# fircarpediem/LSS2_Multimodal_nu

Measured on AMD Instinct MI355X. Metric: BEV frames/sec (6-cam 352x128 -> 200x200x64), full hot path: CamEncode lift + splat + BevEncode, higher is better.
Workload: dtype bf16; 1 GPU; BASELINE configs[1]: model_BEV_TXT LSS hot path, batch=4/GPU, 6 cams 352x128, D=41, 200x200x64 BEV -> BevEncode -> 200x200x4, trunk (EfficientNet) not included: features are the input; batch_per_gpu=4, global_batch=4, parallelism=dp1 (sample-sharded, no collective), precision=bf16

## Files before the change

lss2_multimodal_nu_amd/csrc/conv_ring.hip:

```cpp
#include <type_traits>

#include "conv_launch.h"
#include "lss_device.h"

namespace {

constexpr int RK_SW = 20, RK_SH = 4;
constexpr int RK_PW = 24, RK_PH = 6;
constexpr int RK_KC = 32;
constexpr int RK_POSB = RK_KC * 2;
constexpr int RK_STRIP_PATCH = RK_PH * RK_PW * RK_POSB;
constexpr int RK_SLAB = 128 * RK_KC * 2;
constexpr int RK_SRC_H = 5, RK_SRC_W = 14;
constexpr int RK_SRC_STRIP = RK_SRC_H * RK_SRC_W * RK_POSB;
constexpr int RK_TH = 2 * RK_SH, RK_TW = 2 * RK_SW;
constexpr int RK_TPW = RK_TW + 2, RK_TPH = RK_TH + 2;
constexpr int RK_TPIECE = (RK_TPH * RK_TPW * 4 + 63) / 64;
constexpr int RK_TSRC_H = 7, RK_TSRC_W = 23;
constexpr int RK_TSRC = RK_TSRC_H * RK_TSRC_W * RK_POSB;
constexpr int RK_TSRC_PIECE = (RK_TSRC_H * RK_TSRC_W * 4 + 63) / 64;

struct RingArgs {
  const unsigned short* x;
  const unsigned short* x2;
  const unsigned char* w;
  const float* scale;
  const float* shift;
  unsigned short* y;
  const float* head_w;
  const float* head_b;
  float* head_out;
  int head_n;
  int B, H, W, Cx, C2, up, Hin, Win, Cin, Cout, relu, wt;
  float ry, rx;
  int SX, SY, nstrips, nblk, nch;
  unsigned long long* stats;
};

__device__ __attribute__((aligned(128))) unsigned char lss_ring_zero_page[128];
__device__ int lss_ring_timeouts;

template <int MODE, bool HEAD, int NSL, bool T22>
struct RingLds {
  static constexpr int RING = 0;
  static constexpr int PATCH = NSL * RK_SLAB;
  static constexpr int PBUF = T22 ? RK_TPIECE * 1024 : 4 * RK_STRIP_PATCH;
  static constexpr int SRC = PATCH + 2 * PBUF;
  static constexpr int HEADX = SRC + (MODE == 1 ? (T22 ? RK_TSRC : 4 * RK_SRC_STRIP) : 0);
  static constexpr int FLAGS = HEADX + (HEAD ? 4 * 80 * 4 * 4 : 0);
  static constexpr int TOTAL = FLAGS + 256;
};
constexpr int F_FULL_W = 0, F_FREE_W = 8, F_FULL_P = 16, F_FREE_P = 18, F_HEAD = 20, F_FULL_S = 24, F_FREE_S = 25;

#define RK_TIMEOUT_COUNTER lss_ring_timeouts
#include "ring_prims.h"

typedef __attribute__((ext_vector_type(2))) __bf16 rk_bf16x2;
__device__ __forceinline__ unsigned int rk_pack_bf2(float lo, float hi) {
  const f32x2 v = {lo, hi};
  return __builtin_bit_cast(unsigned int, __builtin_convertvector(v, rk_bf16x2));
}
__device__ __forceinline__ uint4 rk_blend(const uint4& q00, const uint4& q01, const uint4& q10, const uint4& q11,
                                          float lx, float ly) {
  const float w11 = lx * ly, w10 = ly - w11, w01 = lx - w11, w00 = 1.f - lx - ly + w11;
  const unsigned int* u00 = reinterpret_cast<const unsigned int*>(&q00);
  const unsigned int* u01 = reinterpret_cast<const unsigned int*>(&q01);
  const unsigned int* u10 = reinterpret_cast<const unsigned int*>(&q10);
  const unsigned int* u11 = reinterpret_cast<const unsigned int*>(&q11);
  uint4 out;
  unsigned int* o = reinterpret_cast<unsigned int*>(&out);
#pragma unroll
  for (int i = 0; i < 4; ++i) {
    float lo = __builtin_bit_cast(float, u00[i] << 16) * w00;
    float hi = __builtin_bit_cast(float, u00[i] & 0xffff0000u) * w00;
    lo = __builtin_fmaf(__builtin_bit_cast(float, u01[i] << 16), w01, lo);
    hi = __builtin_fmaf(__builtin_bit_cast(float, u01[i] & 0xffff0000u), w01, hi);
    lo = __builtin_fmaf(__builtin_bit_cast(float, u10[i] << 16), w10, lo);
    hi = __builtin_fmaf(__builtin_bit_cast(float, u10[i] & 0xffff0000u), w10, hi);
    lo = __builtin_fmaf(__builtin_bit_cast(float, u11[i] << 16), w11, lo);
    hi = __builtin_fmaf(__builtin_bit_cast(float, u11[i] & 0xffff0000u), w11, hi);
    o[i] = rk_pack_bf2(lo, hi);
  }
  return out;
}

#ifndef RK_PSLEEP
#define RK_PSLEEP 8
#endif
#ifndef RK_PRIO_C
#define RK_PRIO_C 0
#endif
#ifndef RK_PRIO_P
#define RK_PRIO_P 3
#endif
#ifndef RK_PRIO_W
#define RK_PRIO_W 2
#endif
constexpr int RK_NS = 4;
constexpr int RK_NCONS = 2 * RK_NS;
constexpr int RK_NPATCH = 3;
constexpr int RK_NWAVES = RK_NCONS + 1 + RK_NPATCH;

struct RingTile {
  int nb;
  int b[RK_NS], oy0[RK_NS], ox0[RK_NS];
  bool ok[RK_NS];
};

template <int MODE, bool HEAD, int NSL, bool T22>
__global__ __launch_bounds__(RK_NWAVES * 64, 3) void conv_ring_kernel(RingArgs a) {
  static_assert(!T22 || MODE == 1, "shared tile: fused upsample only");
  using L = RingLds<MODE, HEAD, NSL, T22>;
  constexpr int PW = T22 ? RK_TPW : RK_PW;
  constexpr int LA = NSL - 2;
  static_assert(NSL >= 3 && NSL <= 8, "ring depth");
  static_assert(L::TOTAL <= 160 * 1024, "LDS of one CU");
  __shared__ __attribute__((aligned(1024))) unsigned char smem[L::TOTAL];
  const int tid = threadIdx.x, lane = tid & 63;
  const int wave = __builtin_amdgcn_readfirstlane(tid >> 6);
  const rk_flag_t flags = (rk_flag_t)((__attribute__((address_space(3))) unsigned char*)smem + L::FLAGS);
  if (tid < 64) flags[tid] = 0;
  __syncthreads();
  int st0 = 0, st1 = 0;
#ifdef RK_STATS
#define RK_ST(x) x
  const unsigned long long t_entry = a.stats ? __builtin_amdgcn_s_memrealtime() : 0ull;
  auto write_stats = [&]() {
    if (a.stats != nullptr && lane == 0) {
      unsigned long long* o = a.stats + ((size_t)blockIdx.x * RK_NWAVES + wave) * 6;
      o[0] = (unsigned long long)st0; o[1] = (unsigned long long)st1;
      o[2] = __builtin_amdgcn_s_memrealtime() - t_entry; o[3] = t_entry;
    }
  };
#else
#define RK_ST(x)
  auto write_stats = [&]() {};
#endif

  RingTile T;
  {
    const int t = lss_xcd_order(blockIdx.x, gridDim.x);
    T.nb = t % a.nblk;
    const int quad = t / a.nblk;
    if (T22) {
      const int tx = a.SX >> 1, per = tx * (a.SY >> 1);
      const int b = quad / per, rem = quad - b * per, ty = rem / tx;
#pragma unroll
      for (int s = 0; s < RK_NS; ++s) {
        T.ok[s] = true;
        T.b[s] = b;
        T.oy0[s] = ty * RK_TH + (s >> 1) * RK_SH;
        T.ox0[s] = (rem - ty * tx) * RK_TW + (s & 1) * RK_SW;
      }
    } else {
#pragma unroll
      for (int s = 0; s < RK_NS; ++s) {
        int sid = RK_NS * quad + s;
        T.ok[s] = sid < a.nstrips;
        sid = min(sid, a.nstrips - 1);
        const int per = a.SX * a.SY;
        T.b[s] = sid / per;
        const int rem = sid - T.b[s] * per;
        const int sy = rem / a.SX;
        T.oy0[s] = sy * RK_SH;
        T.ox0[s] = (rem - sy * a.SX) * RK_SW;
      }
    }
  }
  const int nsteps = a.nch * 9;

  if (wave == RK_NCONS) {
    __builtin_amdgcn_s_setprio(RK_PRIO_W);
    const unsigned char* wsrc = a.w + (size_t)T.nb * a.nch * 9 * RK_SLAB + lane * 16;
    int slot = 0, gen = 1, pslot = 0, pgen = 1, inflight = 0;
    auto publish_oldest = [&]() {
      switch (inflight) {
        case 1: lss_wait_vmcnt<0>(); break;
        case 2: lss_wait_vmcnt<8>(); break;
        case 3: lss_wait_vmcnt<16>(); break;
        case 4: lss_wait_vmcnt<24>(); break;
        case 5: lss_wait_vmcnt<32>(); break;
        case 6: lss_wait_vmcnt<40>(); break;
        default: lss_wait_vmcnt<48>(); break;
      }
      rk_set(flags + F_FULL_W + pslot, pgen, lane);
      if (++pslot == NSL) { pslot = 0; ++pgen; }
      --inflight;
    };
    for (int i = 0; i < nsteps; ++i) {
      if (gen > 1) {
        int spins = 0;
        while (rk_peek(flags + F_FREE_W + slot) < RK_NCONS * (gen - 1)) {
          if (inflight > 0) {
            publish_oldest();
          } else {
            __builtin_amdgcn_s_sleep(1);
            ++st0;
            if (++spins > RK_SPIN_LIMIT) {
              if (lane == 0) atomicAdd(&lss_ring_timeouts, 1);
              break;
            }
          }
        }
        asm volatile("" ::: "memory");
      }
      unsigned char* dst = smem + L::RING + slot * RK_SLAB;
#ifndef RK_DIAG_NOWDMA
#pragma unroll
      for (int k = 0; k < 8; ++k) lss_glds16(wsrc + (size_t)i * RK_SLAB + k * 1024, dst + k * 1024);
#endif
      ++inflight;
      if (inflight > LA) publish_oldest();
      if (++slot == NSL) { slot = 0; ++gen; }
    }
    while (inflight > 0) publish_oldest();
    lss_wait_vmcnt<0>();
    write_stats();
    return;
  }

  if (wave > RK_NCONS) {
    __builtin_amdgcn_s_setprio(RK_PRIO_P);
    const int pw = wave - RK_NCONS - 1;
    constexpr int NIT = (T22 ? RK_TPIECE : RK_NS * 9) / RK_NPATCH;
    static_assert(NIT * RK_NPATCH == (T22 ? RK_TPIECE : RK_NS * 9), "pieces split evenly over the patch loaders");
    const int nskip = MODE == 1 ? a.C2 / RK_KC : a.nch;
    const unsigned short* xfull = MODE == 1 ? a.x2 : a.x;
    const int cfull = MODE == 1 ? a.C2 : a.Cx;
    int poff[NIT];
    int g_off[MODE == 1 ? NIT : 1];
    constexpr int NWD = MODE == 1 && T22 ? NIT : 1, NWP = MODE == 1 && !T22 ? NIT : 1;
    float g_lx[NWD], g_ly[NWD];
    unsigned int g_wp[NWP];
    constexpr int SRCW = T22 ? RK_TSRC_W : RK_SRC_W;
    constexpr int NSRCP = T22 ? RK_TSRC_PIECE : RK_NS * 5;
    constexpr int NSRC = MODE == 1 ? (NSRCP + RK_NPATCH - 1) / RK_NPATCH : 1;
    int src_o[NSRC];
#pragma unroll
    for (int k = 0; k < NIT; ++k) {
      const int it = pw + k * RK_NPATCH;
      const int s = T22 ? 0 : it / 9, pos = T22 ? it * 16 + (lane >> 2) : (it % 9) * 16 + (lane >> 2);
      const int prow = pos / PW, pcol = pos - prow * PW;
      const int piece = (lane & 3) ^ ((prow & 1) << 1);
      const int sb = s == 0 ? T.b[0] : s == 1 ? T.b[1] : s == 2 ? T.b[2] : T.b[3];
      const int soy = s == 0 ? T.oy0[0] : s == 1 ? T.oy0[1] : s == 2 ? T.oy0[2] : T.oy0[3];
      const int sox = s == 0 ? T.ox0[0] : s == 1 ? T.ox0[1] : s == 2 ? T.ox0[2] : T.ox0[3];
      const bool sok = s == 0 ? T.ok[0] : s == 1 ? T.ok[1] : s == 2 ? T.ok[2] : T.ok[3];
      const int iy = soy - 1 + prow, ix = sox - 1 + pcol;
      const bool used = T22 ? pos < RK_TPH * RK_TPW : pcol < RK_SW + 2;
      const bool in = sok && used && iy >= 0 && iy < a.Hin && ix >= 0 && ix < a.Win;
      poff[k] = (in && cfull > 0) ? ((sb * a.Hin + iy) * a.Win + ix) * cfull + piece * 8 : -1;
      if (MODE == 1) {
        g_off[k] = 0;
        unsigned int g_w = 0;
        if (in) {
          const int wy0 = (int)(a.ry * (float)max(soy - 1, 0)), wx0 = (int)(a.rx * (float)max(sox - 1, 0));
          const float sy = a.ry * (float)iy, sx = a.rx * (float)ix;
          const int y0 = (int)sy, x0 = (int)sx;
          const unsigned int wy = (unsigned int)((sy - (float)y0) * 65536.f + 0.5f);
          const unsigned int wx = (unsigned int)((sx - (float)x0) * 65536.f + 0.5f);
          g_w = min(wx, 65535u) | (min(wy, 65535u) << 16);
          const int fl = (x0 < a.W - 1 ? 1 : 0) | (y0 < a.H - 1 ? 2 : 0) | 4;
          g_off[k] = ((((y0 - wy0) * SRCW + (x0 - wx0)) * 4 + piece) * 16) | fl;
        }
        if constexpr (T22) {
          g_lx[k] = (float)(g_w & 0xffff) * (1.f / 65536.f);
          g_ly[k] = (float)(g_w >> 16) * (1.f / 65536.f);
        } else {
          g_wp[k] = g_w;
        }
      }
    }
    if (MODE == 1) {
#pragma unroll
      for (int k = 0; k < NSRC; ++k) {
        const int it = pw + k * RK_NPATCH;
        const int s = T22 ? 0 : min(it / 5, RK_NS - 1), q = (T22 ? it : it % 5) * 64 + lane;
        const int pos = min(q >> 2, (T22 ? RK_TSRC_H : RK_SRC_H) * SRCW - 1), part = q & 3;
        const int sr = pos / SRCW, sc = pos - sr * SRCW;
        const int sb = s == 0 ? T.b[0] : s == 1 ? T.b[1] : s == 2 ? T.b[2] : T.b[3];
        const int soy = s == 0 ? T.oy0[0] : s == 1 ? T.oy0[1] : s == 2 ? T.oy0[2] : T.oy0[3];
        const int sox = s == 0 ? T.ox0[0] : s == 1 ? T.ox0[1] : s == 2 ? T.ox0[2] : T.ox0[3];
        const int wy0 = (int)(a.ry * (float)max(soy - 1, 0)), wx0 = (int)(a.rx * (float)max(sox - 1, 0));
        src_o[k] = ((sb * a.H + min(wy0 + sr, a.H - 1)) * a.W + min(wx0 + sc, a.W - 1)) * a.Cx + part * 8;
      }
    }
    auto issue_full = [&](int c, int buf) {
      unsigned char* dst = smem + L::PATCH + buf * L::PBUF;
#pragma unroll
      for (int k = 0; k < NIT; ++k) {
        const void* src = poff[k] >= 0 ? (const void*)(xfull + poff[k] + c * RK_KC) : (const void*)lss_ring_zero_page;
        lss_glds16(src, dst + (pw + k * RK_NPATCH) * 1024);
      }
    };
    if (MODE == 0) {
      issue_full(0, 0);
      if (a.nch > 1) {
        issue_full(1, 1);
        lss_wait_vmcnt<NIT>();
      } else {
        lss_wait_vmcnt<0>();
      }
      rk_add1(flags + F_FULL_P + 0, lane);
      for (int c = 0; c < a.nch; ++c) {
        if (c + 1 < a.nch) {
          lss_wait_vmcnt<0>();
          rk_add1(flags + F_FULL_P + ((c + 1) & 1), lane);
        }
        if (c + 2 < a.nch) {
          st0 += rk_wait_ge<RK_PSLEEP>(flags + F_FREE_P + (c & 1), RK_NCONS * ((c >> 1) + 1));
          issue_full(c + 2, c & 1);
        }
      }
    } else {
      auto issue_src = [&](int c) {
        const int cx = c * RK_KC - a.C2;
#pragma unroll
        for (int k = 0; k < NSRC; ++k) {
          const int it = pw + k * RK_NPATCH;
          if (T22) {
            if (it < RK_TSRC_PIECE && it * 64 + lane < RK_TSRC_H * RK_TSRC_W * 4)
              lss_glds16(a.x + src_o[k] + cx, smem + L::SRC + it * 1024);
          } else if (it < RK_NS * 5 && (it % 5) * 64 + lane < RK_SRC_H * RK_SRC_W * 4) {
            lss_glds16(a.x + src_o[k] + cx, smem + L::SRC + (it / 5) * RK_SRC_STRIP + (it % 5) * 1024);
          }
        }
      };
      auto prepare = [&](int c) {
        if (c < nskip) {
          st0 += rk_wait_ge<RK_PSLEEP>(flags + F_FREE_P + (c & 1), RK_NCONS * (c >> 1));
          issue_full(c, c & 1);
        } else {
          st1 += rk_wait_ge(flags + F_FREE_S, RK_NPATCH * (c - nskip));
          issue_src(c);
        }
      };
      prepare(0);
      for (int c = 0; c < a.nch; ++c) {
        lss_wait_vmcnt<0>();
        if (c >= nskip) {
          rk_add1(flags + F_FULL_S, lane);
          st1 += rk_wait_ge(flags + F_FULL_S, RK_NPATCH * (c - nskip + 1));
          st0 += rk_wait_ge<RK_PSLEEP>(flags + F_FREE_P + (c & 1), RK_NCONS * (c >> 1));
          unsigned char* dst = smem + L::PATCH + (c & 1) * L::PBUF;
          uint4 qa[4], qb[4];
          auto corners = [&](int k, uint4* q) {
            const int it = pw + k * RK_NPATCH;
            const unsigned char* p00 = smem + L::SRC + (T22 ? 0 : (it / 9) * RK_SRC_STRIP) + (g_off[k] & 0xfff0);
            const int dx = (g_off[k] & 1) ? 4 * 16 : 0, dy = (g_off[k] & 2) ? SRCW * 4 * 16 : 0;
            q[0] = *reinterpret_cast<const uint4*>(p00);
#if defined(RK_DIAG_ONEREAD)
            q[1] = q[0]; q[2] = q[0]; q[3] = q[0];
            asm volatile("" : "+v"(q[1].x), "+v"(q[2].x), "+v"(q[3].x));
#else
            q[1] = *reinterpret_cast<const uint4*>(p00 + dx);
            q[2] = *reinterpret_cast<const uint4*>(p00 + dy);
            q[3] = *reinterpret_cast<const uint4*>(p00 + dy + dx);
#endif
          };
          auto finish = [&](int k, const uint4* q) {
            uint4 v = make_uint4(0, 0, 0, 0);
#ifndef RK_DIAG_NOBLEND
#if defined(RK_DIAG_READSONLY)
            v.x = q[0].x ^ q[1].x ^ q[2].x ^ q[3].x; v.y = q[0].y ^ q[1].y ^ q[2].y ^ q[3].y;
            v.z = q[0].z ^ q[1].z ^ q[2].z ^ q[3].z; v.w = q[0].w ^ q[1].w ^ q[2].w ^ q[3].w;
#else
            if constexpr (T22)
              v = rk_blend(q[0], q[1], q[2], q[3], g_lx[k], g_ly[k]);
            else
              v = rk_blend(q[0], q[1], q[2], q[3], (float)(g_wp[k] & 0xffff) * (1.f / 65536.f),
                           (float)(g_wp[k] >> 16) * (1.f / 65536.f));
#endif
            const bool in = (g_off[k] & 4) != 0;
            v.x = in ? v.x : 0u; v.y = in ? v.y : 0u; v.z = in ? v.z : 0u; v.w = in ? v.w : 0u;
#endif
            *reinterpret_cast<uint4*>(dst + (pw + k * RK_NPATCH) * 1024 + lane * 16) = v;
          };
          corners(0, qa);
#pragma unroll
          for (int k = 0; k < NIT; k += 2) {
            if (k + 1 < NIT) corners(k + 1, qb);
            finish(k, qa);
            if (k + 1 < NIT) {
              if (k + 2 < NIT) corners(k + 2, qa);
              finish(k + 1, qb);
            }
          }
          lss_wait_lgkm0();
          rk_add1(flags + F_FREE_S, lane);
        }
        if (c + 1 < a.nch && c + 1 >= nskip) prepare(c + 1);
        rk_add1(flags + F_FULL_P + (c & 1), lane);
        if (c + 1 < a.nch && c + 1 < nskip) prepare(c + 1);
      }
    }
    lss_wait_vmcnt<0>();
    write_stats();
    return;
  }

  __builtin_amdgcn_s_setprio(RK_PRIO_C);
  const int sidx = wave >> 1, cg = wave & 1;
  const int n = lane & 15, kq = lane >> 4;
  const int my_b = sidx == 0 ? T.b[0] : sidx == 1 ? T.b[1] : sidx == 2 ? T.b[2] : T.b[3];
  const int my_oy0 = sidx == 0 ? T.oy0[0] : sidx == 1 ? T.oy0[1] : sidx == 2 ? T.oy0[2] : T.oy0[3];
  const int my_ox0 = sidx == 0 ? T.ox0[0] : sidx == 1 ? T.ox0[1] : sidx == 2 ? T.ox0[2] : T.ox0[3];
  const bool my_ok = sidx == 0 ? T.ok[0] : sidx == 1 ? T.ok[1] : sidx == 2 ? T.ok[2] : T.ok[3];
  f32x4 acc[5][4];
#pragma unroll
  for (int j = 0; j < 5; ++j)
#pragma unroll
    for (int t = 0; t < 4; ++t) acc[j][t] = (f32x4){0.f, 0.f, 0.f, 0.f};
  bf16x8 fw[4], fp[5];
#define RK_DSR(dst, addr, off) asm volatile("ds_read_b128 %0, %1 offset:%2" : "=v"(dst) : "v"(addr), "n"(off))
  const unsigned int lanepk =
      (unsigned int)(cg * 4096 + lane * 16) |
      ((unsigned int)((((n >> 2) * PW + (n & 3)) * RK_POSB + (kq << 4)) ^ (((n >> 2) & 1) << 5)) << 16);
  const unsigned int flag_base = (unsigned int)(__UINTPTR_TYPE__)flags;
  const int pconst = L::PATCH + (T22 ? ((sidx >> 1) * RK_SH * PW + (sidx & 1) * RK_SW) * RK_POSB : sidx * RK_STRIP_PATCH);
  auto add1 = [&](int word) {
    unsigned long long save;
    asm volatile("s_mov_b64 %0, exec\n\ts_mov_b64 exec, 1\n\tds_add_u32 %1, %2\n\ts_mov_b64 exec, %0"
                 : "=&s"(save)
                 : "v"(flag_base + 4 * word), "v"(1)
                 : "memory");
  };

  RK_ST(const unsigned long long tc_loop = __builtin_amdgcn_s_memtime(); const unsigned long long tr_loop = __builtin_amdgcn_s_memrealtime();)
  int slot = 0, gen = 1, buf = 0, pgen = 1;
  rk_wait_ge(flags + F_FULL_P + 0, RK_NPATCH);
  rk_wait_ge(flags + F_FULL_W + 0, 1);
  int fnext;
  {
    const int wa = (int)(lanepk & 0xffffu) + L::RING, pa = (int)(lanepk >> 16) + pconst;
    RK_DSR(fw[0], wa, 0);
    RK_DSR(fw[1], wa, 1024);
    asm volatile("ds_read_b32 %0, %1" : "=v"(fnext) : "v"(flag_base + 4 * (F_FULL_W + (1 % NSL))));
    RK_DSR(fp[0], pa, 0 * 4 * RK_POSB);
    RK_DSR(fp[1], pa, 1 * 4 * RK_POSB);
    RK_DSR(fp[2], pa, 2 * 4 * RK_POSB);
    RK_DSR(fp[3], pa, 3 * 4 * RK_POSB);
    RK_DSR(fp[4], pa, 4 * 4 * RK_POSB);
  }

  auto step = [&](auto TAPc, bool last) {
    constexpr int TAP = decltype(TAPc)::value;
    constexpr int NT = (TAP + 1) % 9;
    constexpr int POFF = (NT / 3) * (PW * RK_POSB) + (NT % 3) * RK_POSB;
    {
      const int wa = (int)(lanepk & 0xffffu) + (L::RING + slot * RK_SLAB);
      RK_DSR(fw[2], wa, 2048);
      RK_DSR(fw[3], wa, 3072);
    }
    __builtin_amdgcn_sched_barrier(0);
    asm volatile("s_waitcnt lgkmcnt(6)" : "+v"(fw[0]), "+v"(fw[1]), "+v"(fp[0]));
    acc[0][0] = __builtin_amdgcn_mfma_f32_16x16x32_bf16(fw[0], fp[0], acc[0][0], 0, 0, 0);
    acc[0][1] = __builtin_amdgcn_mfma_f32_16x16x32_bf16(fw[1], fp[0], acc[0][1], 0, 0, 0);
    __builtin_amdgcn_sched_barrier(0);
    int nslot = slot + 1, ngen = gen;
    if (nslot == NSL) { nslot = 0; ++ngen; }
    int nbuf = buf, npgen = pgen;
    if (TAP == 8) {
      nbuf = buf ^ 1;
      if (nbuf == 0) ++npgen;
    }
    const int wan = (int)(lanepk & 0xffffu) + (L::RING + nslot * RK_SLAB);
    __builtin_amdgcn_sched_barrier(0);
    asm volatile("s_waitcnt lgkmcnt(5)" : "+v"(fp[1]));
    acc[1][0] = __builtin_amdgcn_mfma_f32_16x16x32_bf16(fw[0], fp[1], acc[1][0], 0, 0, 0);
    acc[1][1] = __builtin_amdgcn_mfma_f32_16x16x32_bf16(fw[1], fp[1], acc[1][1], 0, 0, 0);
    __builtin_amdgcn_sched_barrier(0);
    const int pan = (int)((lanepk >> 16) ^ (NT / 3 == 1 ? 32u : 0u)) + (pconst + nbuf * L::PBUF);
    const int n2 = nslot + 1 == NSL ? 0 : nslot + 1;
    const unsigned int fa = flag_base + 4 * (F_FULL_W + n2);
    __builtin_amdgcn_sched_barrier(0);
    asm volatile("s_waitcnt lgkmcnt(4)" : "+v"(fp[2]));
    acc[2][0] = __builtin_amdgcn_mfma_f32_16x16x32_bf16(fw[0], fp[2], acc[2][0], 0, 0, 0);
    acc[2][1] = __builtin_amdgcn_mfma_f32_16x16x32_bf16(fw[1], fp[2], acc[2][1], 0, 0, 0);
    __builtin_amdgcn_sched_barrier(0);
    asm volatile("s_waitcnt lgkmcnt(3)" : "+v"(fp[3]));
    acc[3][0] = __builtin_amdgcn_mfma_f32_16x16x32_bf16(fw[0], fp[3], acc[3][0], 0, 0, 0);
    acc[3][1] = __builtin_amdgcn_mfma_f32_16x16x32_bf16(fw[1], fp[3], acc[3][1], 0, 0, 0);
    __builtin_amdgcn_sched_barrier(0);
    asm volatile("s_waitcnt lgkmcnt(2)" : "+v"(fp[4]));
    acc[4][0] = __builtin_amdgcn_mfma_f32_16x16x32_bf16(fw[0], fp[4], acc[4][0], 0, 0, 0);
    acc[4][1] = __builtin_amdgcn_mfma_f32_16x16x32_bf16(fw[1], fp[4], acc[4][1], 0, 0, 0);
    __builtin_amdgcn_sched_barrier(0);
    if (!last) {
      if (__builtin_amdgcn_readfirstlane(fnext) < ngen) st0 += 1 + rk_wait_ge(flags + F_FULL_W + nslot, ngen);
      if (TAP == 8) st1 += rk_wait_ge(flags + F_FULL_P + nbuf, RK_NPATCH * npgen);
      asm volatile("" ::: "memory");
      RK_DSR(fw[0], wan, 0);
      RK_DSR(fw[1], wan, 1024);
      asm volatile("ds_read_b32 %0, %1" : "=v"(fnext) : "v"(fa));
      __builtin_amdgcn_sched_barrier(0);
      asm volatile("s_waitcnt lgkmcnt(3)" : "+v"(fw[2]), "+v"(fw[3]));
    } else {
      asm volatile("s_waitcnt lgkmcnt(0)" : "+v"(fw[2]), "+v"(fw[3]));
    }
    acc[0][2] = __builtin_amdgcn_mfma_f32_16x16x32_bf16(fw[2], fp[0], acc[0][2], 0, 0, 0);
    acc[0][3] = __builtin_amdgcn_mfma_f32_16x16x32_bf16(fw[3], fp[0], acc[0][3], 0, 0, 0);
    __builtin_amdgcn_sched_barrier(0);
    add1(F_FREE_W + slot);
    if (!last) RK_DSR(fp[0], pan, POFF + 0 * 4 * RK_POSB);
    __builtin_amdgcn_sched_barrier(0);
    acc[1][2] = __builtin_amdgcn_mfma_f32_16x16x32_bf16(fw[2], fp[1], acc[1][2], 0, 0, 0);
    acc[1][3] = __builtin_amdgcn_mfma_f32_16x16x32_bf16(fw[3], fp[1], acc[1][3], 0, 0, 0);
    __builtin_amdgcn_sched_barrier(0);
    if (!last) RK_DSR(fp[1], pan, POFF + 1 * 4 * RK_POSB);
    __builtin_amdgcn_sched_barrier(0);
    acc[2][2] = __builtin_amdgcn_mfma_f32_16x16x32_bf16(fw[2], fp[2], acc[2][2], 0, 0, 0);
    acc[2][3] = __builtin_amdgcn_mfma_f32_16x16x32_bf16(fw[3], fp[2], acc[2][3], 0, 0, 0);
    __builtin_amdgcn_sched_barrier(0);
    if (!last) RK_DSR(fp[2], pan, POFF + 2 * 4 * RK_POSB);
    __builtin_amdgcn_sched_barrier(0);
    acc[3][2] = __builtin_amdgcn_mfma_f32_16x16x32_bf16(fw[2], fp[3], acc[3][2], 0, 0, 0);
    acc[3][3] = __builtin_amdgcn_mfma_f32_16x16x32_bf16(fw[3], fp[3], acc[3][3], 0, 0, 0);
    __builtin_amdgcn_sched_barrier(0);
    if (!last) RK_DSR(fp[3], pan, POFF + 3 * 4 * RK_POSB);
    __builtin_amdgcn_sched_barrier(0);
    acc[4][2] = __builtin_amdgcn_mfma_f32_16x16x32_bf16(fw[2], fp[4], acc[4][2], 0, 0, 0);
    acc[4][3] = __builtin_amdgcn_mfma_f32_16x16x32_bf16(fw[3], fp[4], acc[4][3], 0, 0, 0);
    __builtin_amdgcn_sched_barrier(0);
    if (!last) RK_DSR(fp[4], pan, POFF + 4 * 4 * RK_POSB);
    if (TAP == 8) add1(F_FREE_P + buf);
    __builtin_amdgcn_sched_barrier(0);
    slot = nslot; gen = ngen; buf = nbuf; pgen = npgen;
  };
  for (int c = 0; c < a.nch; ++c) {
    step(std::integral_constant<int, 0>{}, false);
    step(std::integral_constant<int, 1>{}, false);
    step(std::integral_constant<int, 2>{}, false);
    step(std::integral_constant<int, 3>{}, false);
    step(std::integral_constant<int, 4>{}, false);
    step(std::integral_constant<int, 5>{}, false);
    step(std::integral_constant<int, 6>{}, false);
    step(std::integral_constant<int, 7>{}, false);
    step(std::integral_constant<int, 8>{}, c + 1 == a.nch);
  }
#undef RK_DSR
  RK_ST(if (a.stats != nullptr && lane == 0) { unsigned long long* o = a.stats + ((size_t)blockIdx.x * RK_NWAVES + wave) * 6; o[2] = __builtin_amdgcn_s_memrealtime() - t_entry; o[4] = __builtin_amdgcn_s_memtime() - tc_loop; o[5] = __builtin_amdgcn_s_memrealtime() - tr_loop; })

  const int ch0 = T.nb * 128 + cg * 64 + kq * 16;
  {
    float sc[16], sh[16];
#pragma unroll
    for (int v4 = 0; v4 < 4; ++v4) {
      f32x4 s4 = {1.f, 1.f, 1.f, 1.f}, h4 = {0.f, 0.f, 0.f, 0.f};
      if (a.scale) s4 = *reinterpret_cast<const f32x4*>(a.scale + ch0 + v4 * 4);
      if (a.shift) h4 = *reinterpret_cast<const f32x4*>(a.shift + ch0 + v4 * 4);
#pragma unroll
      for (int i = 0; i < 4; ++i) { sc[v4 * 4 + i] = s4[i]; sh[v4 * 4 + i] = h4[i]; }
    }
#pragma unroll
    for (int j = 0; j < 5; ++j)
#pragma unroll
      for (int t = 0; t < 4; ++t)
#pragma unroll
        for (int i = 0; i < 4; ++i) {
          float v = acc[j][t][i] * sc[t * 4 + i] + sh[t * 4 + i];
          acc[j][t][i] = a.relu ? fmaxf(v, 0.f) : v;
        }
  }
  const int oy = my_oy0 + (n >> 2);
  if (!HEAD) {
    const __amdgpu_buffer_rsrc_t yrsrc = __builtin_amdgcn_make_buffer_rsrc(
        a.y, 0, a.wt ? (int)((size_t)a.B * a.Hin * a.Win * a.Cout * 2) : 0, 0x00020000);
    const int chs = T.nb * 128 + cg * 64 + kq * 8;
#pragma unroll
    for (int j = 0; j < 5; ++j) {
      const int ox = my_ox0 + j * 4 + (n & 3);
      u32x4 ox_[2];
#pragma unroll
      for (int d = 0; d < 4; ++d) {
        const unsigned lo = rk_pack_bf2(acc[j][d >> 1][(d & 1) * 2], acc[j][d >> 1][(d & 1) * 2 + 1]);
        const unsigned hi = rk_pack_bf2(acc[j][2 + (d >> 1)][(d & 1) * 2], acc[j][2 + (d >> 1)][(d & 1) * 2 + 1]);
        const u32x2 r = __builtin_amdgcn_permlane16_swap(lo, hi, false, false);
        const u32x2 t = __builtin_amdgcn_permlane32_swap(r[0], r[1], false, false);
        ox_[0][d] = t[0];
        ox_[1][d] = t[1];
      }
      if (!my_ok || oy >= a.Hin || ox >= a.Win) continue;
      const size_t o = (((size_t)my_b * a.Hin + oy) * a.Win + ox) * a.Cout + chs;
#pragma unroll
      for (int hf = 0; hf < 2; ++hf) {
        if (a.wt) __builtin_amdgcn_raw_buffer_store_b128(ox_[hf], yrsrc, (int)((o + hf * 32) * 2), 0, 16);
        else *reinterpret_cast<u32x4*>(a.y + o + hf * 32) = ox_[hf];
      }
    }
  } else {
    float part[5];
#pragma unroll
    for (int j = 0; j < 5; ++j) part[j] = 0.f;
    const int c0 = cg * 64 + kq * 16;
#pragma unroll 1
    for (int k = 0; k < 4; ++k) {
      float hw[16];
#pragma unroll
      for (int v4 = 0; v4 < 4; ++v4) {
        f32x4 w4 = {0.f, 0.f, 0.f, 0.f};
        if (k < a.head_n) w4 = *reinterpret_cast<const f32x4*>(a.head_w + (size_t)k * 128 + c0 + v4 * 4);
#pragma unroll
        for (int i = 0; i < 4; ++i) hw[v4 * 4 + i] = w4[i];
      }
#pragma unroll
      for (int j = 0; j < 5; ++j) {
        float s = 0.f;
#pragma unroll
        for (int t = 0; t < 4; ++t)
#pragma unroll
          for (int i = 0; i < 4; ++i) s = fmaf(acc[j][t][i], hw[t * 4 + i], s);
        s += __shfl_xor(s, 16, 64);
        s += __shfl_xor(s, 32, 64);
        if (kq == k) part[j] = s;
      }
    }
    float* hx = reinterpret_cast<float*>(smem + L::HEADX) + sidx * (80 * 4);
    if (cg == 1) {
#pragma unroll
      for (int j = 0; j < 5; ++j) hx[(j * 16 + n) * 4 + kq] = part[j];
      lss_wait_lgkm0();
      rk_set(flags + F_HEAD + sidx, 1, lane);
    } else {
      rk_wait_ge(flags + F_HEAD + sidx, 1);
      if (kq < a.head_n) {
        const float hb = a.head_b[kq];
#pragma unroll
        for (int j = 0; j < 5; ++j) {
          const int ox = my_ox0 + j * 4 + (n & 3);
          const float v = part[j] + hx[(j * 16 + n) * 4 + kq] + hb;
          if (my_ok && oy < a.Hin && ox < a.Win)
            a.head_out[(((size_t)my_b * a.head_n + kq) * a.Hin + oy) * a.Win + ox] = v;
        }
      }
    }
  }
  RK_ST(if (a.stats != nullptr && lane == 0) {
    unsigned long long* o = a.stats + ((size_t)blockIdx.x * RK_NWAVES + wave) * 6;
    o[0] = (unsigned long long)st0; o[1] = (unsigned long long)st1; o[3] = t_entry;
  })
#undef RK_ST
}

template <bool DGRAD>
__global__ void pack_weights_ring_kernel(const float* __restrict__ w, int Cout, int Cin, unsigned short* __restrict__ out) {
  const size_t n = (size_t)Cout * Cin * 9;
  const int nch = Cin / RK_KC;
  for (size_t e = (size_t)blockIdx.x * 256 + threadIdx.x; e < n; e += (size_t)gridDim.x * 256) {
    const int j = e & 7;
    size_t r = e >> 3;
    const int l = r & 63; r >>= 6;
    const int t = r & 3; r >>= 2;
    const int cg = r & 1; r >>= 1;
    const int tap = r % 9; r /= 9;
    const int chunk = r % nch;
    const int nb = r / nch;
    const int co = nb * 128 + cg * 64 + ((l & 15) >> 2) * 16 + 4 * t + (l & 3);
    const int ci = chunk * RK_KC + (l >> 4) * 8 + j;
    out[e] = lss_f2bf(DGRAD ? w[((size_t)ci * Cout + co) * 9 + (8 - tap)] : w[((size_t)co * Cin + ci) * 9 + tap]);
  }
}

}

extern "C" int lss_conv2d_ring_ok(int B, int H, int W, int Cx, int C2, int up, int Cout, int head_n) {
  if (B <= 0 || H <= 0 || W <= 0 || Cx <= 0 || C2 < 0 || up <= 0 || Cout <= 0 || head_n < 0) return 0;
  if (Cout % 128 != 0 || Cx % 32 != 0 || C2 % 32 != 0) return 0;
  if (head_n > 0 && (Cout != 128 || head_n > 4)) return 0;
  const bool fused = up > 1 || C2 > 0;
  const int Hin = H * up, Win = W * up;
  if (fused) {
    if (up < 2) return 0;
    const float ry = Hin > 1 ? (float)(H - 1) / (float)(Hin - 1) : 0.f, rx = Win > 1 ? (float)(W - 1) / (float)(Win - 1) : 0.f;
    if ((int)(ry * (RK_PH - 1) + 0.999f) + 2 > RK_SRC_H || (int)(rx * (RK_SW + 1) + 0.999f) + 2 > RK_SRC_W) return 0;
  }
  if ((long long)B * Hin * Win * (long long)Cout >= (1LL << 31) / 2) return 0;
  if ((long long)B * H * W * (long long)Cx >= (1LL << 31) || (long long)B * Hin * Win * (long long)(C2 > 0 ? C2 : 1) >= (1LL << 31))
    return 0;
  const long long strips = (long long)B * lss_cdiv(Hin, RK_SH) * lss_cdiv(Win, RK_SW);
  return strips / RK_NS * (Cout / 128) >= 96 ? 1 : 0;
}

extern "C" int lss_conv2d_ring_timeouts(void) {
  int v = -1;
  if (hipMemcpyFromSymbol(&v, HIP_SYMBOL(lss_ring_timeouts), sizeof(int), 0, hipMemcpyDeviceToHost) != hipSuccess) return -1;
  return v;
}

extern "C" size_t lss_conv2d_ring_packed_weight_bytes(int Cout, int Cin) {
  if (Cout <= 0 || Cin <= 0 || Cout % 128 != 0 || Cin % RK_KC != 0) return 0;
  return (size_t)Cout * Cin * 9 * 2;
}

extern "C" int lss_conv2d_pack_weights_ring(const float* w_oihw, int Cout, int Cin, void* w_packed, void* stream) {
  LSS_CHECK_PTR(w_oihw); LSS_CHECK_PTR(w_packed);
  if (lss_conv2d_ring_packed_weight_bytes(Cout, Cin) == 0) return LSS_E_SHAPE;
  const size_t n = (size_t)Cout * Cin * 9;
  const int grid = (int)((n + 255) / 256 > 4096 ? 4096 : (n + 255) / 256);
  hipLaunchKernelGGL(pack_weights_ring_kernel<false>, dim3(grid), dim3(256), 0, lss_stream(stream), w_oihw, Cout, Cin,
                     reinterpret_cast<unsigned short*>(w_packed));
  return lss_launch_status();
}

extern "C" int lss_conv2d_pack_weights_ring_dgrad(const float* w_oihw, int Cout, int Cin, void* w_packed, void* stream) {
  LSS_CHECK_PTR(w_oihw); LSS_CHECK_PTR(w_packed);
  if (lss_conv2d_ring_packed_weight_bytes(Cin, Cout) == 0) return LSS_E_SHAPE;
  const size_t n = (size_t)Cout * Cin * 9;
  const int grid = (int)((n + 255) / 256 > 4096 ? 4096 : (n + 255) / 256);
  hipLaunchKernelGGL(pack_weights_ring_kernel<true>, dim3(grid), dim3(256), 0, lss_stream(stream), w_oihw, Cin, Cout,
                     reinterpret_cast<unsigned short*>(w_packed));
  return lss_launch_status();
}

int lss_conv_ring_launch(const void* x, const void* x2, const void* w_ring, const float* scale, const float* shift,
                         void* y, const float* head_w, const float* head_b, float* head_out, int head_n, int B, int H,
                         int W, int Cx, int C2, int up, int Cout, int relu, int wt, hipStream_t st) {
  if (!lss_conv2d_ring_ok(B, H, W, Cx, C2, up, Cout, head_n)) return LSS_E_SHAPE;
  if (relu != 0 && relu != 1) return LSS_E_LAYOUT;
  RingArgs a;
  a.x = reinterpret_cast<const unsigned short*>(x);
  a.x2 = reinterpret_cast<const unsigned short*>(x2);
  a.w = reinterpret_cast<const unsigned char*>(w_ring);
  a.scale = scale; a.shift = shift;
  a.y = reinterpret_cast<unsigned short*>(y);
  a.head_w = head_w; a.head_b = head_b; a.head_out = head_out; a.head_n = head_n;
  a.B = B; a.H = H; a.W = W; a.Cx = Cx; a.C2 = C2; a.up = up;
  a.Hin = H * up; a.Win = W * up; a.Cin = Cx + C2; a.Cout = Cout; a.relu = relu; a.wt = wt;
  a.ry = a.Hin > 1 ? (float)(H - 1) / (float)(a.Hin - 1) : 0.f;
  a.rx = a.Win > 1 ? (float)(W - 1) / (float)(a.Win - 1) : 0.f;
  a.SX = lss_cdiv(a.Win, RK_SW); a.SY = lss_cdiv(a.Hin, RK_SH);
  a.nstrips = B * a.SX * a.SY;
  a.nblk = Cout / 128;
  a.nch = a.Cin / RK_KC;
  a.stats = lss_env_device_ptr("LSS_RING_STATS");
  const bool fused = up > 1 || C2 > 0;
  const bool t22 = fused && a.Hin % RK_TH == 0 && a.Win % RK_TW == 0 &&
                   (int)(a.ry * (RK_TPH - 1) + 0.999f) + 2 <= RK_TSRC_H && (int)(a.rx * (RK_TPW - 1) + 0.999f) + 2 <= RK_TSRC_W;
  const dim3 g((a.nstrips + RK_NS - 1) / RK_NS * a.nblk), blk(RK_NWAVES * 64);
  if (head_n > 0) {
    if (t22) hipLaunchKernelGGL((conv_ring_kernel<1, true, 7, true>), g, blk, 0, st, a);
    else if (fused) hipLaunchKernelGGL((conv_ring_kernel<1, true, 7, false>), g, blk, 0, st, a);
    else hipLaunchKernelGGL((conv_ring_kernel<0, true, 8, false>), g, blk, 0, st, a);
  } else {
    if (t22) hipLaunchKernelGGL((conv_ring_kernel<1, false, 7, true>), g, blk, 0, st, a);
    else if (fused) hipLaunchKernelGGL((conv_ring_kernel<1, false, 7, false>), g, blk, 0, st, a);
    else hipLaunchKernelGGL((conv_ring_kernel<0, false, 8, false>), g, blk, 0, st, a);
  }
  return lss_launch_status();
}
```

Before: 12260 frames/s.

## Group weight ring slots into three-slab tap rows to cut consumer handshakes

Adds an SPS template parameter. With SPS=3, each weight-ring slot holds a full 3x3 tap row of three slabs, and the ring is three slots deep, so one ring cycle covers one input chunk. Consumers now wait on full flags and signal free flags once per three taps instead of every tap. They use constant LDS offsets per tap instead of recomputing slot addresses, and the producer issues 24 DMA pieces per fill. It also moves the MFMAs and flag atomics to inline asm with scalar-held addresses and adds nops for accumulator hazards. The cost is coarser producer/consumer granularity, which can expose more weight-load latency, and a changed LDS footprint.

```diff
diff --git a/lss2_multimodal_nu_amd/csrc/conv_ring.hip b/lss2_multimodal_nu_amd/csrc/conv_ring.hip
--- a/lss2_multimodal_nu_amd/csrc/conv_ring.hip
+++ b/lss2_multimodal_nu_amd/csrc/conv_ring.hip
@@ -40,10 +40,10 @@
 __device__ __attribute__((aligned(128))) unsigned char lss_ring_zero_page[128];
 __device__ int lss_ring_timeouts;
 
-template <int MODE, bool HEAD, int NSL, bool T22>
+template <int MODE, bool HEAD, int NSL, bool T22, int SPS>
 struct RingLds {
   static constexpr int RING = 0;
-  static constexpr int PATCH = NSL * RK_SLAB;
+  static constexpr int PATCH = NSL * SPS * RK_SLAB;
   static constexpr int PBUF = T22 ? RK_TPIECE * 1024 : 4 * RK_STRIP_PATCH;
   static constexpr int SRC = PATCH + 2 * PBUF;
   static constexpr int HEADX = SRC + (MODE == 1 ? (T22 ? RK_TSRC : 4 * RK_SRC_STRIP) : 0);
@@ -107,13 +107,16 @@
   bool ok[RK_NS];
 };
 
-template <int MODE, bool HEAD, int NSL, bool T22>
+template <int MODE, bool HEAD, int NSL, bool T22, int SPS>
 __global__ __launch_bounds__(RK_NWAVES * 64, 3) void conv_ring_kernel(RingArgs a) {
   static_assert(!T22 || MODE == 1, "shared tile: fused upsample only");
-  using L = RingLds<MODE, HEAD, NSL, T22>;
+  using L = RingLds<MODE, HEAD, NSL, T22, SPS>;
   constexpr int PW = T22 ? RK_TPW : RK_PW;
   constexpr int LA = NSL - 2;
+  constexpr int SLOTB = SPS * RK_SLAB, NPC = SPS * 8;
   static_assert(NSL >= 3 && NSL <= 8, "ring depth");
+  static_assert(SPS == 1 || (SPS == 3 && NSL == 3), "a three-slab slot is a tap row and the ring one chunk");
+  static_assert((LA + 1) * NPC < 64, "the pieces in flight must fit the 6-bit vmcnt");
   static_assert(L::TOTAL <= 160 * 1024, "LDS of one CU");
   __shared__ __attribute__((aligned(1024))) unsigned char smem[L::TOTAL];
   const int tid = threadIdx.x, lane = tid & 63;
@@ -174,20 +177,26 @@
     const unsigned char* wsrc = a.w + (size_t)T.nb * a.nch * 9 * RK_SLAB + lane * 16;
     int slot = 0, gen = 1, pslot = 0, pgen = 1, inflight = 0;
     auto publish_oldest = [&]() {
-      switch (inflight) {
-        case 1: lss_wait_vmcnt<0>(); break;
-        case 2: lss_wait_vmcnt<8>(); break;
-        case 3: lss_wait_vmcnt<16>(); break;
-        case 4: lss_wait_vmcnt<24>(); break;
-        case 5: lss_wait_vmcnt<32>(); break;
-        case 6: lss_wait_vmcnt<40>(); break;
-        default: lss_wait_vmcnt<48>(); break;
+      if constexpr (SPS == 3) {
+        if (inflight == 1) lss_wait_vmcnt<0>();
+        else lss_wait_vmcnt<NPC>();
+      } else {
+        switch (inflight) {
+          case 1: lss_wait_vmcnt<0>(); break;
+          case 2: lss_wait_vmcnt<8>(); break;
+          case 3: lss_wait_vmcnt<16>(); break;
+          case 4: lss_wait_vmcnt<24>(); break;
+          case 5: lss_wait_vmcnt<32>(); break;
+          case 6: lss_wait_vmcnt<40>(); break;
+          default: lss_wait_vmcnt<48>(); break;
+        }
       }
       rk_set(flags + F_FULL_W + pslot, pgen, lane);
       if (++pslot == NSL) { pslot = 0; ++pgen; }
       --inflight;
     };
-    for (int i = 0; i < nsteps; ++i) {
+    const int nfill = nsteps / SPS;
+    for (int i = 0; i < nfill; ++i) {
       if (gen > 1) {
         int spins = 0;
         while (rk_peek(flags + F_FREE_W + slot) < RK_NCONS * (gen - 1)) {
@@ -204,10 +213,10 @@
         }
         asm volatile("" ::: "memory");
       }
-      unsigned char* dst = smem + L::RING + slot * RK_SLAB;
+      unsigned char* dst = smem + L::RING + slot * SLOTB;
 #ifndef RK_DIAG_NOWDMA
 #pragma unroll
-      for (int k = 0; k < 8; ++k) lss_glds16(wsrc + (size_t)i * RK_SLAB + k * 1024, dst + k * 1024);
+      for (int k = 0; k < NPC; ++k) lss_glds16(wsrc + (size_t)i * SLOTB + k * 1024, dst + k * 1024);
 #endif
       ++inflight;
       if (inflight > LA) publish_oldest();
@@ -401,7 +410,7 @@
 
   __builtin_amdgcn_s_setprio(RK_PRIO_C);
   const int sidx = wave >> 1, cg = wave & 1;
-  const int n = lane & 15, kq = lane >> 4;
+  const int n0 = lane & 15, kq0 = lane >> 4;
   const int my_b = sidx == 0 ? T.b[0] : sidx == 1 ? T.b[1] : sidx == 2 ? T.b[2] : T.b[3];
   const int my_oy0 = sidx == 0 ? T.oy0[0] : sidx == 1 ? T.oy0[1] : sidx == 2 ? T.oy0[2] : T.oy0[3];
   const int my_ox0 = sidx == 0 ? T.ox0[0] : sidx == 1 ? T.ox0[1] : sidx == 2 ? T.ox0[2] : T.ox0[3];
@@ -413,29 +422,45 @@
     for (int t = 0; t < 4; ++t) acc[j][t] = (f32x4){0.f, 0.f, 0.f, 0.f};
   bf16x8 fw[4], fp[5];
 #define RK_DSR(dst, addr, off) asm volatile("ds_read_b128 %0, %1 offset:%2" : "=v"(dst) : "v"(addr), "n"(off))
+#define RK_MFMA(c, wf, pf)                                                                                   \
+  do {                                                                                                       \
+    if constexpr (SPS == 3) asm volatile("v_mfma_f32_16x16x32_bf16 %0, %1, %2, %0" : "+v"(c) : "v"(wf), "v"(pf)); \
+    else c = __builtin_amdgcn_mfma_f32_16x16x32_bf16(wf, pf, c, 0, 0, 0);                                    \
+  } while (0)
   const unsigned int lanepk =
       (unsigned int)(cg * 4096 + lane * 16) |
-      ((unsigned int)((((n >> 2) * PW + (n & 3)) * RK_POSB + (kq << 4)) ^ (((n >> 2) & 1) << 5)) << 16);
+      ((unsigned int)((((n0 >> 2) * PW + (n0 & 3)) * RK_POSB + (kq0 << 4)) ^ (((n0 >> 2) & 1) << 5)) << 16);
   const unsigned int flag_base = (unsigned int)(__UINTPTR_TYPE__)flags;
   const int pconst = L::PATCH + (T22 ? ((sidx >> 1) * RK_SH * PW + (sidx & 1) * RK_SW) * RK_POSB : sidx * RK_STRIP_PATCH);
   auto add1 = [&](int word) {
     unsigned long long save;
-    asm volatile("s_mov_b64 %0, exec\n\ts_mov_b64 exec, 1\n\tds_add_u32 %1, %2\n\ts_mov_b64 exec, %0"
-                 : "=&s"(save)
-                 : "v"(flag_base + 4 * word), "v"(1)
-                 : "memory");
+    if constexpr (SPS == 1) {
+      asm volatile("s_mov_b64 %0, exec\n\ts_mov_b64 exec, 1\n\tds_add_u32 %1, %2\n\ts_mov_b64 exec, %0"
+                   : "=&s"(save)
+                   : "v"(flag_base + 4 * word), "v"(1)
+                   : "memory");
+    } else {
+      unsigned int ta, tb;
+      asm volatile("s_mov_b64 %0, exec\n\ts_mov_b64 exec, 1\n\tv_mov_b32 %1, %3\n\tv_mov_b32 %2, 1\n\t"
+                   "ds_add_u32 %1, %2\n\ts_mov_b64 exec, %0"
+                   : "=&s"(save), "=&v"(ta), "=&v"(tb)
+                   : "s"(flag_base + 4 * word)
+                   : "memory");
+    }
   };
 
   RK_ST(const unsigned long long tc_loop = __builtin_amdgcn_s_memtime(); const unsigned long long tr_loop = __builtin_amdgcn_s_memrealtime();)
   int slot = 0, gen = 1, buf = 0, pgen = 1;
   rk_wait_ge(flags + F_FULL_P + 0, RK_NPATCH);
   rk_wait_ge(flags + F_FULL_W + 0, 1);
-  int fnext;
+  int fnext = 0;
+  const int wbase = (int)(lanepk & 0xffffu) + L::RING;
+  int w8 = 0;
   {
     const int wa = (int)(lanepk & 0xffffu) + L::RING, pa = (int)(lanepk >> 16) + pconst;
     RK_DSR(fw[0], wa, 0);
     RK_DSR(fw[1], wa, 1024);
-    asm volatile("ds_read_b32 %0, %1" : "=v"(fnext) : "v"(flag_base + 4 * (F_FULL_W + (1 % NSL))));
+    if constexpr (SPS == 1) asm volatile("ds_read_b32 %0, %1" : "=v"(fnext) : "v"(flag_base + 4 * (F_FULL_W + (1 % NSL))));
     RK_DSR(fp[0], pa, 0 * 4 * RK_POSB);
     RK_DSR(fp[1], pa, 1 * 4 * RK_POSB);
     RK_DSR(fp[2], pa, 2 * 4 * RK_POSB);
@@ -447,80 +472,116 @@
     constexpr int TAP = decltype(TAPc)::value;
     constexpr int NT = (TAP + 1) % 9;
     constexpr int POFF = (NT / 3) * (PW * RK_POSB) + (NT % 3) * RK_POSB;
-    {
+    constexpr bool SLOT_END = SPS == 1 || TAP % 3 == 2;
+    constexpr bool FLAG_RD = SPS == 1 || TAP % 3 == 1;
+    if constexpr (SPS == 1) {
       const int wa = (int)(lanepk & 0xffffu) + (L::RING + slot * RK_SLAB);
       RK_DSR(fw[2], wa, 2048);
       RK_DSR(fw[3], wa, 3072);
+    } else if constexpr (TAP < 8) {
+      RK_DSR(fw[2], wbase, TAP * RK_SLAB + 2048);
+      RK_DSR(fw[3], wbase, TAP * RK_SLAB + 3072);
+    } else {
+      RK_DSR(fw[2], w8, 2048);
+      RK_DSR(fw[3], w8, 3072);
     }
     __builtin_amdgcn_sched_barrier(0);
     asm volatile("s_waitcnt lgkmcnt(6)" : "+v"(fw[0]), "+v"(fw[1]), "+v"(fp[0]));
-    acc[0][0] = __builtin_amdgcn_mfma_f32_16x16x32_bf16(fw[0], fp[0], acc[0][0], 0, 0, 0);
-    acc[0][1] = __builtin_amdgcn_mfma_f32_16x16x32_bf16(fw[1], fp[0], acc[0][1], 0, 0, 0);
-    __builtin_amdgcn_sched_barrier(0);
-    int nslot = slot + 1, ngen = gen;
-    if (nslot == NSL) { nslot = 0; ++ngen; }
+    RK_MFMA(acc[0][0], fw[0], fp[0]);
+    RK_MFMA(acc[0][1], fw[1], fp[0]);
+    __builtin_amdgcn_sched_barrier(0);
+    int nslot = slot, ngen = gen;
+    if constexpr (SPS == 1) {
+      if (++nslot == NSL) { nslot = 0; ++ngen; }
+    } else {
+      if (TAP == 8) ++ngen;
+    }
     int nbuf = buf, npgen = pgen;
     if (TAP == 8) {
       nbuf = buf ^ 1;
       if (nbuf == 0) ++npgen;
     }
-    const int wan = (int)(lanepk & 0xffffu) + (L::RING + nslot * RK_SLAB);
+    int wan = 0;
+    if constexpr (SPS == 1) wan = (int)(lanepk & 0xffffu) + (L::RING + nslot * RK_SLAB);
+    else if constexpr (NT == 8) asm volatile("v_add_u32 %0, 0x10000, %1" : "=v"(w8) : "v"(wbase));
     __builtin_amdgcn_sched_barrier(0);
     asm volatile("s_waitcnt lgkmcnt(5)" : "+v"(fp[1]));
-    acc[1][0] = __builtin_amdgcn_mfma_f32_16x16x32_bf16(fw[0], fp[1], acc[1][0], 0, 0, 0);
-    acc[1][1] = __builtin_amdgcn_mfma_f32_16x16x32_bf16(fw[1], fp[1], acc[1][1], 0, 0, 0);
+    RK_MFMA(acc[1][0], fw[0], fp[1]);
+    RK_MFMA(acc[1][1], fw[1], fp[1]);
     __builtin_amdgcn_sched_barrier(0);
     const int pan = (int)((lanepk >> 16) ^ (NT / 3 == 1 ? 32u : 0u)) + (pconst + nbuf * L::PBUF);
-    const int n2 = nslot + 1 == NSL ? 0 : nslot + 1;
-    const unsigned int fa = flag_base + 4 * (F_FULL_W + n2);
+    unsigned int fa = 0;
+    if constexpr (SPS == 1) {
+      const int n2 = nslot + 1 == NSL ? 0 : nslot + 1;
+      fa = flag_base + 4 * (F_FULL_W + n2);
+    } else if constexpr (FLAG_RD) {
+      fa = flag_base + 4 * (F_FULL_W + (TAP / 3 + 1) % 3);
+    }
     __builtin_amdgcn_sched_barrier(0);
     asm volatile("s_waitcnt lgkmcnt(4)" : "+v"(fp[2]));
-    acc[2][0] = __builtin_amdgcn_mfma_f32_16x16x32_bf16(fw[0], fp[2], acc[2][0], 0, 0, 0);
-    acc[2][1] = __builtin_amdgcn_mfma_f32_16x16x32_bf16(fw[1], fp[2], acc[2][1], 0, 0, 0);
+    RK_MFMA(acc[2][0], fw[0], fp[2]);
+    RK_MFMA(acc[2][1], fw[1], fp[2]);
     __builtin_amdgcn_sched_barrier(0);
     asm volatile("s_waitcnt lgkmcnt(3)" : "+v"(fp[3]));
-    acc[3][0] = __builtin_amdgcn_mfma_f32_16x16x32_bf16(fw[0], fp[3], acc[3][0], 0, 0, 0);
-    acc[3][1] = __builtin_amdgcn_mfma_f32_16x16x32_bf16(fw[1], fp[3], acc[3][1], 0, 0, 0);
+    RK_MFMA(acc[3][0], fw[0], fp[3]);
+    RK_MFMA(acc[3][1], fw[1], fp[3]);
     __builtin_amdgcn_sched_barrier(0);
     asm volatile("s_waitcnt lgkmcnt(2)" : "+v"(fp[4]));
-    acc[4][0] = __builtin_amdgcn_mfma_f32_16x16x32_bf16(fw[0], fp[4], acc[4][0], 0, 0, 0);
-    acc[4][1] = __builtin_amdgcn_mfma_f32_16x16x32_bf16(fw[1], fp[4], acc[4][1], 0, 0, 0);
+    RK_MFMA(acc[4][0], fw[0], fp[4]);
+    RK_MFMA(acc[4][1], fw[1], fp[4]);
     __builtin_amdgcn_sched_barrier(0);
     if (!last) {
-      if (__builtin_amdgcn_readfirstlane(fnext) < ngen) st0 += 1 + rk_wait_ge(flags + F_FULL_W + nslot, ngen);
+      if constexpr (SLOT_END) {
+        if (__builtin_amdgcn_readfirstlane(fnext) < ngen)
+          st0 += 1 + rk_wait_ge(flags + F_FULL_W + (SPS == 1 ? nslot : NT / 3), ngen);
+      }
       if (TAP == 8) st1 += rk_wait_ge(flags + F_FULL_P + nbuf, RK_NPATCH * npgen);
       asm volatile("" ::: "memory");
-      RK_DSR(fw[0], wan, 0);
-      RK_DSR(fw[1], wan, 1024);
-      asm volatile("ds_read_b32 %0, %1" : "=v"(fnext) : "v"(fa));
-      __builtin_amdgcn_sched_barrier(0);
-      asm volatile("s_waitcnt lgkmcnt(3)" : "+v"(fw[2]), "+v"(fw[3]));
+      if constexpr (SPS == 1) {
+        RK_DSR(fw[0], wan, 0);
+        RK_DSR(fw[1], wan, 1024);
+      } else if constexpr (NT < 8) {
+        RK_DSR(fw[0], wbase, NT * RK_SLAB + 0);
+        RK_DSR(fw[1], wbase, NT * RK_SLAB + 1024);
+      } else {
+        RK_DSR(fw[0], w8, 0);
+        RK_DSR(fw[1], w8, 1024);
+      }
+      if constexpr (FLAG_RD) {
+        if constexpr (SPS == 1) asm volatile("ds_read_b32 %0, %1" : "=v"(fnext) : "v"(fa));
+        else asm volatile("v_mov_b32 %0, %1\n\tds_read_b32 %0, %0" : "=&v"(fnext) : "s"(fa));
+        __builtin_amdgcn_sched_barrier(0);
+        asm volatile("s_waitcnt lgkmcnt(3)" : "+v"(fw[2]), "+v"(fw[3]));
+      } else {
+        __builtin_amdgcn_sched_barrier(0);
+        asm volatile("s_waitcnt lgkmcnt(2)" : "+v"(fw[2]), "+v"(fw[3]));
+      }
     } else {
       asm volatile("s_waitcnt lgkmcnt(0)" : "+v"(fw[2]), "+v"(fw[3]));
     }
-    acc[0][2] = __builtin_amdgcn_mfma_f32_16x16x32_bf16(fw[2], fp[0], acc[0][2], 0, 0, 0);
-    acc[0][3] = __builtin_amdgcn_mfma_f32_16x16x32_bf16(fw[3], fp[0], acc[0][3], 0, 0, 0);
-    __builtin_amdgcn_sched_barrier(0);
-    add1(F_FREE_W + slot);
+    RK_MFMA(acc[0][2], fw[2], fp[0]);
+    RK_MFMA(acc[0][3], fw[3], fp[0]);
+    __builtin_amdgcn_sched_barrier(0);
+    if constexpr (SLOT_END) add1(F_FREE_W + (SPS == 1 ? slot : TAP / 3));
     if (!last) RK_DSR(fp[0], pan, POFF + 0 * 4 * RK_POSB);
     __builtin_amdgcn_sched_barrier(0);
-    acc[1][2] = __builtin_amdgcn_mfma_f32_16x16x32_bf16(fw[2], fp[1], acc[1][2], 0, 0, 0);
-    acc[1][3] = __builtin_amdgcn_mfma_f32_16x16x32_bf16(fw[3], fp[1], acc[1][3], 0, 0, 0);
+    RK_MFMA(acc[1][2], fw[2], fp[1]);
+    RK_MFMA(acc[1][3], fw[3], fp[1]);
     __builtin_amdgcn_sched_barrier(0);
     if (!last) RK_DSR(fp[1], pan, POFF + 1 * 4 * RK_POSB);
     __builtin_amdgcn_sched_barrier(0);
-    acc[2][2] = __builtin_amdgcn_mfma_f32_16x16x32_bf16(fw[2], fp[2], acc[2][2], 0, 0, 0);
-    acc[2][3] = __builtin_amdgcn_mfma_f32_16x16x32_bf16(fw[3], fp[2], acc[2][3], 0, 0, 0);
+    RK_MFMA(acc[2][2], fw[2], fp[2]);
+    RK_MFMA(acc[2][3], fw[3], fp[2]);
     __builtin_amdgcn_sched_barrier(0);
     if (!last) RK_DSR(fp[2], pan, POFF + 2 * 4 * RK_POSB);
     __builtin_amdgcn_sched_barrier(0);
-    acc[3][2] = __builtin_amdgcn_mfma_f32_16x16x32_bf16(fw[2], fp[3], acc[3][2], 0, 0, 0);
-    acc[3][3] = __builtin_amdgcn_mfma_f32_16x16x32_bf16(fw[3], fp[3], acc[3][3], 0, 0, 0);
+    RK_MFMA(acc[3][2], fw[2], fp[3]);
+    RK_MFMA(acc[3][3], fw[3], fp[3]);
     __builtin_amdgcn_sched_barrier(0);
     if (!last) RK_DSR(fp[3], pan, POFF + 3 * 4 * RK_POSB);
     __builtin_amdgcn_sched_barrier(0);
-    acc[4][2] = __builtin_amdgcn_mfma_f32_16x16x32_bf16(fw[2], fp[4], acc[4][2], 0, 0, 0);
-    acc[4][3] = __builtin_amdgcn_mfma_f32_16x16x32_bf16(fw[3], fp[4], acc[4][3], 0, 0, 0);
+    RK_MFMA(acc[4][2], fw[2], fp[4]);
+    RK_MFMA(acc[4][3], fw[3], fp[4]);
     __builtin_amdgcn_sched_barrier(0);
     if (!last) RK_DSR(fp[4], pan, POFF + 4 * 4 * RK_POSB);
     if (TAP == 8) add1(F_FREE_P + buf);
@@ -539,8 +600,17 @@
     step(std::integral_constant<int, 8>{}, c + 1 == a.nch);
   }
 #undef RK_DSR
+#undef RK_MFMA
+  if constexpr (SPS == 3) {
+#define RK_A(j) "+v"(acc[j][0]), "+v"(acc[j][1]), "+v"(acc[j][2]), "+v"(acc[j][3])
+    asm volatile("s_nop 15\n\ts_nop 15" : RK_A(0), RK_A(1), RK_A(2), RK_A(3), RK_A(4));
+#undef RK_A
+  }
   RK_ST(if (a.stats != nullptr && lane == 0) { unsigned long long* o = a.stats + ((size_t)blockIdx.x * RK_NWAVES + wave) * 6; o[2] = __builtin_amdgcn_s_memrealtime() - t_entry; o[4] = __builtin_amdgcn_s_memtime() - tc_loop; o[5] = __builtin_amdgcn_s_memrealtime() - tr_loop; })
 
+  int lane_e = lane;
+  if constexpr (SPS == 3) asm volatile("v_mbcnt_lo_u32_b32 %0, -1, 0\n\tv_mbcnt_hi_u32_b32 %0, -1, %0" : "=v"(lane_e));
+  const int n = lane_e & 15, kq = lane_e >> 4;
   const int ch0 = T.nb * 128 + cg * 64 + kq * 16;
   {
     float sc[16], sh[16];
@@ -620,7 +690,7 @@
 #pragma unroll
       for (int j = 0; j < 5; ++j) hx[(j * 16 + n) * 4 + kq] = part[j];
       lss_wait_lgkm0();
-      rk_set(flags + F_HEAD + sidx, 1, lane);
+      rk_set(flags + F_HEAD + sidx, 1, lane_e);
     } else {
       rk_wait_ge(flags + F_HEAD + sidx, 1);
       if (kq < a.head_n) {
@@ -738,13 +808,13 @@
                    (int)(a.ry * (RK_TPH - 1) + 0.999f) + 2 <= RK_TSRC_H && (int)(a.rx * (RK_TPW - 1) + 0.999f) + 2 <= RK_TSRC_W;
   const dim3 g((a.nstrips + RK_NS - 1) / RK_NS * a.nblk), blk(RK_NWAVES * 64);
   if (head_n > 0) {
-    if (t22) hipLaunchKernelGGL((conv_ring_kernel<1, true, 7, true>), g, blk, 0, st, a);
-    else if (fused) hipLaunchKernelGGL((conv_ring_kernel<1, true, 7, false>), g, blk, 0, st, a);
-    else hipLaunchKernelGGL((conv_ring_kernel<0, true, 8, false>), g, blk, 0, st, a);
+    if (t22) hipLaunchKernelGGL((conv_ring_kernel<1, true, 3, true, 3>), g, blk, 0, st, a);
+    else if (fused) hipLaunchKernelGGL((conv_ring_kernel<1, true, 7, false, 1>), g, blk, 0, st, a);
+    else hipLaunchKernelGGL((conv_ring_kernel<0, true, 3, false, 3>), g, blk, 0, st, a);
   } else {
-    if (t22) hipLaunchKernelGGL((conv_ring_kernel<1, false, 7, true>), g, blk, 0, st, a);
-    else if (fused) hipLaunchKernelGGL((conv_ring_kernel<1, false, 7, false>), g, blk, 0, st, a);
-    else hipLaunchKernelGGL((conv_ring_kernel<0, false, 8, false>), g, blk, 0, st, a);
+    if (t22) hipLaunchKernelGGL((conv_ring_kernel<1, false, 3, true, 3>), g, blk, 0, st, a);
+    else if (fused) hipLaunchKernelGGL((conv_ring_kernel<1, false, 7, false, 1>), g, blk, 0, st, a);
+    else hipLaunchKernelGGL((conv_ring_kernel<0, false, 3, false, 3>), g, blk, 0, st, a);
   }
   return lss_launch_status();
 }
```

Result: faster. 12490 frames/s, median of 6 (+1.9%).
